# dohlee/chromoformer

Measured on AMD Instinct MI355X. Metric: genes/sec training (bsz=64, default config), higher is better.
Workload: dtype f32

## Files before the change

chromoformer_amd/csrc/cf_attc1.h:

```cpp
#pragma once

namespace cf {

__host__ __device__ inline size_t attc1_smem(int L, int F) {
    const int Lpad = attc2_lpad(L);
    return (size_t)(2 * kD + 16 + 16 + kD * 8 + ((L * F + 8 + 3) & ~3) + 2 * (Lpad + 4) + 2 * Lpad + 64 + 16 * 2 * kD) * sizeof(float) + (size_t)Lpad;
}

#define CF_STAMP1(slot)                                                                                   \
    do {                                                                                                  \
        if (a.tdbg && stamp_wg == 0 && threadIdx.x == 0)                                                   \
            a.tdbg[(BWD ? 16 : 0) + (slot)] = __builtin_amdgcn_s_memtime();                               \
    } while (0)
template <bool BWD>
__device__ __forceinline__ void attc1_body(const Attc2Args& a, const int r, const int n, float* smem, const int stamp_wg = -1) {
    const int tid = threadIdx.x;
    const int w = tid >> 6, lane = tid & 63;
    const int L = a.L[r], Lpad = a.Lpad[r], LT = a.LT[r], F = a.F, LS = Lpad + 4;
    float* vin_s = smem;
    float* u_s = vin_s + 2 * kD;
    float* w_s = u_s + 16;
    float* wlp_s = w_s + 16;
    float* feats_s = wlp_s + kD * 8;
    float* sc_s = feats_s + ((L * F + 8 + 3) & ~3);
    float* p_s = sc_s + 2 * LS;
    float* red_s = p_s + 2 * Lpad;
    float* part_s = red_s + 64;
    uint8_t* mk_s = reinterpret_cast<uint8_t*>(part_s + 16 * 2 * kD);

    CF_STAMP1(0);
    const int eg = tid >> 7, j4 = tid & 127;
    float4 tb[16];
    {
        const float* fg = a.feats[r] + (size_t)n * L * F;
        const uint8_t* mg = a.mask[r] + (size_t)n * a.mstride[r];
        const float wl0 = (tid & 7) < F ? ldg(a.wlp[r] + (tid >> 3) * F + (tid & 7)) : 0.f;
        const float wl1 = (tid & 7) < F ? ldg(a.wlp[r] + ((tid + kAT) >> 3) * F + (tid & 7)) : 0.f;
        float4 vv = make_float4(0.f, 0.f, 0.f, 0.f);
        if (tid < 64) vv = ldg4(a.vin[r] + (size_t)n * 256 + tid * 4);
        uint8_t mb[2];
#pragma unroll
        for (int u = 0; u < 2; ++u) {
            const int j = tid + u * kAT;
            mb[u] = *(const CF_GLOBAL uint8_t*)(mg + min(j, L - 1));
        }
        float pb[4];
        if (BWD) {
            const float* pg = a.p[r] + (size_t)n * 2 * L;
#pragma unroll
            for (int u = 0; u < 4; ++u) {
                const int i = tid + u * kAT, h = i / Lpad, j = i - h * Lpad;
                pb[u] = ldg(pg + min(h, 1) * L + min(j, L - 1));
            }
        }
        float fb[8];
        const int nfe = L * F;
#pragma unroll
        for (int u = 0; u < 8; ++u) fb[u] = ldg(fg + min(tid + u * kAT, nfe - 1));
        {
            const float* pt = a.pet[r] + (size_t)(eg * 32) * LT + min(4 * j4, LT - 4);
#pragma unroll
            for (int k = 0; k < 16; ++k) tb[k] = ldg4(pt + (size_t)k * LT);
        }
        __builtin_amdgcn_sched_barrier(0);
        wlp_s[tid] = wl0;
        wlp_s[tid + kAT] = wl1;
        if (tid < 64) *reinterpret_cast<float4*>(vin_s + tid * 4) = vv;
#pragma unroll
        for (int u = 0; u < 2; ++u)
            if (tid + u * kAT < Lpad) mk_s[tid + u * kAT] = tid + u * kAT < L ? mb[u] : (uint8_t)1;
        if (BWD)
#pragma unroll
            for (int u = 0; u < 4; ++u)
                if (tid + u * kAT < 2 * Lpad) p_s[tid + u * kAT] = (tid + u * kAT) % Lpad < L ? pb[u] : 0.f;
#pragma unroll
        for (int u = 0; u < 8; ++u)
            if (tid + u * kAT < nfe + 8) feats_s[tid + u * kAT] = tid + u * kAT < nfe ? fb[u] : 0.f;
        for (int i = tid + 8 * kAT; i < nfe + 8; i += kAT) feats_s[i] = i < nfe ? ldg(fg + i) : 0.f;
        for (int i = tid; i < 2 * LS; i += kAT) {
            const int j = i % LS;
            if (j >= L) sc_s[i] = 0.f;
        }
    }
    __syncthreads();
    CF_STAMP1(1);
    {
        const int o = tid >> 5, part = tid & 31, h = o >> 3, f = o & 7;
        float acc = 0.f;
#pragma unroll
        for (int i = 0; i < 4; ++i) acc = fmaf(vin_s[h * kD + part * 4 + i], wlp_s[(part * 4 + i) * 8 + f], acc);
        acc = group16_sum(acc);
        acc += __shfl_xor(acc, 16, 64);
        if (part == 0) u_s[o] = acc;
    }
    float t0[2] = {0.f, 0.f}, t1[2] = {0.f, 0.f};
    for (int c = 0; c * kAT < L; ++c) {
        const int jc = min(c * kAT + 4 * j4, LT - 4);
        const float* pt = a.pet[r] + (size_t)(eg * 32) * LT + jc;
        float4 s0 = make_float4(0.f, 0.f, 0.f, 0.f), s1 = s0;
#pragma unroll
        for (int half = 0; half < 2; ++half) {
            float4 b[16];
            if (c == 0) {
#pragma unroll
                for (int k = 0; k < 16; ++k) b[k] = tb[k];
                if (half == 0) {
#pragma unroll
                    for (int k = 0; k < 16; ++k) tb[k] = ldg4(pt + (size_t)(16 + k) * LT);
                }
            } else {
#pragma unroll
                for (int k = 0; k < 16; ++k) b[k] = ldg4(pt + (size_t)(half * 16 + k) * LT);
            }
#pragma unroll
            for (int k4 = 0; k4 < 4; ++k4) {
                const float4 v0 = *reinterpret_cast<const float4*>(vin_s + eg * 32 + half * 16 + 4 * k4);
                const float4 v1 = *reinterpret_cast<const float4*>(vin_s + kD + eg * 32 + half * 16 + 4 * k4);
                const float q0[4] = {v0.x, v0.y, v0.z, v0.w}, q1[4] = {v1.x, v1.y, v1.z, v1.w};
#pragma unroll
                for (int i = 0; i < 4; ++i) {
                    const float4 bb = b[4 * k4 + i];
                    s0 = make_float4(fmaf(q0[i], bb.x, s0.x), fmaf(q0[i], bb.y, s0.y), fmaf(q0[i], bb.z, s0.z), fmaf(q0[i], bb.w, s0.w));
                    s1 = make_float4(fmaf(q1[i], bb.x, s1.x), fmaf(q1[i], bb.y, s1.y), fmaf(q1[i], bb.z, s1.z), fmaf(q1[i], bb.w, s1.w));
                }
            }
        }
        if (c) __syncthreads();
        *reinterpret_cast<float4*>(part_s + (eg * 2) * kAT + 4 * j4) = s0;
        *reinterpret_cast<float4*>(part_s + (eg * 2 + 1) * kAT + 4 * j4) = s1;
        __syncthreads();
        t0[c] = (part_s[tid] + part_s[2 * kAT + tid]) + (part_s[4 * kAT + tid] + part_s[6 * kAT + tid]);
        t1[c] = (part_s[kAT + tid] + part_s[3 * kAT + tid]) + (part_s[5 * kAT + tid] + part_s[7 * kAT + tid]);
    }
    const int e4 = tid & 31, jg = tid >> 5;
    const int per5 = (L + 15) / 16;
    const int j05 = jg * per5, nj5 = max(0, min(L, j05 + per5) - j05);
    const float* pp5 = a.pe[r] + (size_t)min(j05, Lpad - 1) * kD + 4 * e4;
#pragma unroll
    for (int k = 0; k < 16; ++k) tb[k] = ldg4(pp5 + (size_t)min(k, max(nj5 - 1, 0)) * kD);
    __syncthreads();
    CF_STAMP1(2);
    auto block_reduce = [&](float v0, float v1, bool is_max, float& o0, float& o1) {
        v0 = is_max ? wave_max(v0) : wave_sum(v0);
        v1 = is_max ? wave_max(v1) : wave_sum(v1);
        __syncthreads();
        if (lane == 0) {
            red_s[w * 2] = v0;
            red_s[w * 2 + 1] = v1;
        }
        __syncthreads();
        o0 = red_s[0];
        o1 = red_s[1];
#pragma unroll
        for (int k = 1; k < kAT / 64; ++k) {
            o0 = is_max ? fmaxf(o0, red_s[k * 2]) : o0 + red_s[k * 2];
            o1 = is_max ? fmaxf(o1, red_s[k * 2 + 1]) : o1 + red_s[k * 2 + 1];
        }
    };
    {
        float x0[2], x1[2];
        bool valid[2], masked[2];
#pragma unroll
        for (int c = 0; c < 2; ++c) {
            const int j = tid + c * kAT;
            valid[c] = j < L;
            masked[c] = valid[c] && mk_s[min(j, Lpad - 1)];
            float f0 = 0.f, f1 = 0.f;
// ... 31 lines not shown
            const float r0 = 1.0f / Z0, r1 = 1.0f / Z1;
            float* pg = a.p[r] + (size_t)n * 2 * L;
#pragma unroll
            for (int c = 0; c < 2; ++c) {
                const int j = tid + c * kAT;
                if (valid[c]) {
                    const float p0 = x0[c] * r0, p1 = x1[c] * r1;
                    sc_s[j] = p0;
                    sc_s[LS + j] = p1;
                    stg(pg + j, p0);
                    stg(pg + L + j, p1);
                }
            }
        } else {
            float d0 = 0.f, d1 = 0.f;
#pragma unroll
            for (int c = 0; c < 2; ++c) {
                const int j = tid + c * kAT;
                if (valid[c]) {
                    d0 = fmaf(p_s[j], x0[c], d0);
                    d1 = fmaf(p_s[Lpad + j], x1[c], d1);
                }
            }
            float D0, D1;
            block_reduce(d0, d1, false, D0, D1);
#pragma unroll
            for (int c = 0; c < 2; ++c) {
                const int j = tid + c * kAT;
                if (valid[c]) {
                    sc_s[j] = masked[c] ? 0.f : p_s[j] * (x0[c] - D0) * a.rscale;
                    sc_s[LS + j] = masked[c] ? 0.f : p_s[Lpad + j] * (x1[c] - D1) * a.rscale;
                }
            }
        }
    }
    __syncthreads();
    CF_STAMP1(3);
    {
        const int o = tid >> 5, part = tid & 31, h = o >> 3, f = o & 7;
        float acc = 0.f;
        if (f < F)
            for (int j = part; j < L; j += 32) acc = fmaf(sc_s[h * LS + j], feats_s[(size_t)j * F + f], acc);
        acc = group16_sum(acc);
        acc += __shfl_xor(acc, 16, 64);
        if (part == 0) {
            w_s[o] = acc;
            stg(a.w[r] + (size_t)n * 16 + o, acc);
        }
    }
    CF_STAMP1(4);
    CF_STAMP1(5);
    {
        float4 o0 = make_float4(0.f, 0.f, 0.f, 0.f), o1 = o0;
        for (int jb = 0; jb < nj5; jb += 16) {
            float4 b[16];
#pragma unroll
            for (int k = 0; k < 16; ++k) b[k] = tb[k];
            if (jb + 16 < nj5) {
#pragma unroll
                for (int k = 0; k < 16; ++k) tb[k] = ldg4(pp5 + (size_t)min(jb + 16 + k, nj5 - 1) * kD);
            }
#pragma unroll
            for (int k = 0; k < 16; ++k) {
                const bool in = jb + k < nj5;
                const float ph = in ? sc_s[j05 + jb + k] : 0.f, qh = in ? sc_s[LS + j05 + jb + k] : 0.f;
                o0 = make_float4(fmaf(ph, b[k].x, o0.x), fmaf(ph, b[k].y, o0.y), fmaf(ph, b[k].z, o0.z), fmaf(ph, b[k].w, o0.w));
                o1 = make_float4(fmaf(qh, b[k].x, o1.x), fmaf(qh, b[k].y, o1.y), fmaf(qh, b[k].z, o1.z), fmaf(qh, b[k].w, o1.w));
            }
        }
        __syncthreads();
        *reinterpret_cast<float4*>(part_s + (jg * 2) * kD + 4 * e4) = o0;
        *reinterpret_cast<float4*>(part_s + (jg * 2 + 1) * kD + 4 * e4) = o1;
    }
    __syncthreads();
    CF_STAMP1(6);
    if (tid < 2 * kD) {
        const int h = tid >> 7, e = tid & 127;
        float v = 0.f;
#pragma unroll
        for (int g = 0; g < 16; ++g) v += part_s[(g * 2 + h) * kD + e];
#pragma unroll
        for (int f = 0; f < 8; ++f) v = fmaf(w_s[h * 8 + f], wlp_s[e * 8 + f], v);
        stg(a.vout[r] + (size_t)n * 256 + tid, v);
    }
    CF_STAMP1(7);
}
template <bool BWD>
__global__ __launch_bounds__(kAT) void k_attc1(Attc2Args a) {
    extern __shared__ __attribute__((aligned(16))) float smem[];
    attc1_body<BWD>(a, gridDim.y - 1 - blockIdx.y, blockIdx.x, smem, blockIdx.y * gridDim.x + blockIdx.x);
}

}
```

chromoformer_amd/csrc/cf_attc2.h:

```cpp
#pragma once
#include <type_traits>

namespace cf {

struct Attc2Args {
    const float* feats[kMaxRes];
    const uint8_t* mask[kMaxRes];
    long long mstride[kMaxRes];
    const float* pe[kMaxRes];
    const float* pet[kMaxRes];
    const float* wlp[kMaxRes];
    const float* vin[kMaxRes];
    float* p[kMaxRes];
    float* w[kMaxRes];
    float* vout[kMaxRes];
    int L[kMaxRes], Lpad[kMaxRes], LT[kMaxRes];
    int N, F;
    float scale, rscale;
    unsigned long long* tdbg;
    unsigned long long* tall;
};
#define CF_STAMP2(slot)                                                                                   \
    do {                                                                                                  \
        if (a.tdbg && stamp_wg == 0 && (threadIdx.x & 63) == 0)                                            \
// ... 9 lines not shown

__device__ __forceinline__ void frag_load_nn_rt(FragNN<4, 8>& f, const float* __restrict__ Bm, int ldb, int nchunks) {
    const int lane = threadIdx.x & 63, r = lane & 15, q = lane >> 4;
    f.bp = Bm + (size_t)(q * 4) * ldb + 4 * r;
    f.ldb = ldb;
#pragma unroll
    for (int c = 0; c < kRing - 1; ++c) frag_chunk_nn(f, c, min(c, nchunks - 1));
    __builtin_amdgcn_sched_barrier(0);
}
__device__ __forceinline__ void frag_mma_nn_rt(FragNN<4, 8>& f, const float* As, int lda, int nchunks, f32x4 (&acc)[4]) {
    const int lane = threadIdx.x & 63, r = lane & 15, q = lane >> 4;
    const float* ap = As + r * lda + q * 4;
    float4 a_nxt = *reinterpret_cast<const float4*>(ap);
    for (int c0 = 0; c0 < nchunks; c0 += kRing) {
#pragma unroll
        for (int u = 0; u < kRing; ++u) {
            const int c = c0 + u;
            if (c + kRing - 1 < nchunks) frag_chunk_nn(f, (u + kRing - 1) % kRing, c + kRing - 1);
            __builtin_amdgcn_sched_barrier(0);
            if (c < nchunks)
#pragma unroll
                for (int k = 0; k < 2; ++k) {
                    const float4 a = a_nxt;
                    a_nxt = *reinterpret_cast<const float4*>(ap + (c * 2 + k + 1) * 16);
                    const float av[4] = {a.x, a.y, a.z, a.w};
#pragma unroll
                    for (int i = 0; i < 4; ++i) {
                        const float* bv = reinterpret_cast<const float*>(&f.ring[u][k][i]);
#pragma unroll
                        for (int t = 0; t < 4; ++t) acc[t] = mfma4(av[i], bv[t], acc[t]);
                    }
                }
        }
    }
}

__host__ __device__ inline size_t attc2_scratch_floats(int L) { return (size_t)kTile * (attc2_lpad(L) + 4) + 2 * kTile * (kD + 4) + 2 * kTile * 8; }
__host__ __device__ inline size_t attc2_persist_bytes(int L, int F, int AG) {
    return (size_t)(kD * 8 + AG * L * F + 8) * sizeof(float) + (size_t)AG * attc2_lpad(L);
}
template <int AG>
__device__ __forceinline__ void attc2_stage(const float* feats, const uint8_t* mask, long long mstride, const float* wlp, int L, int Lpad, int F,
                                            const int n0, const int N, float* persist) {
    const int tid = threadIdx.x, w = __builtin_amdgcn_readfirstlane(tid >> 6);
    float* wlp_s = persist;
    float* feats_s = wlp_s + kD * 8;
    uint8_t* mk_s = reinterpret_cast<uint8_t*>(feats_s + AG * L * F + 8);
    const int nreg = min(AG, N - n0);
    const float* fg = feats + (size_t)n0 * L * F;
    const int nf = nreg * L * F;
    constexpr int NFL = AG == 8 ? 12 : AG == 4 ? 6 : AG == 2 ? 3 : 2;
    const bool f16b = ((L * F) & 3) == 0 && AG * L * F <= NFL * 4 * kAT && (reinterpret_cast<uintptr_t>(fg) & 15) == 0;
    if (f16b) {
        const int n4 = (AG * L * F) >> 2, last4 = (nf >> 2) - 1;
#pragma unroll
        for (int u = 0; u < NFL; ++u) {
            const int i = tid + u * kAT;
            typedef __attribute__((address_space(3))) void* lds_void;
            typedef const __attribute__((address_space(1))) void* glb_void;
            if (i < n4)
                __builtin_amdgcn_global_load_lds((glb_void)(fg + (size_t)min(i, last4) * 4), (lds_void)(feats_s + (size_t)(w * 64 + u * kAT) * 4), 16, 0, 0);
        }
    } else {
        for (int i = tid; i < AG * L * F; i += kAT) feats_s[i] = i < nf ? ldg(fg + i) : 0.f;
    }
    if (tid < 8) feats_s[AG * L * F + tid] = 0.f;
    static_assert(kD * 8 == 2 * kAT, "wlp staging assumes two entries per thread");
    wlp_s[tid] = (tid & 7) < F ? ldg(wlp + (tid >> 3) * F + (tid & 7)) : 0.f;
    wlp_s[tid + kAT] = (tid & 7) < F ? ldg(wlp + ((tid + kAT) >> 3) * F + (tid & 7)) : 0.f;
    const uint8_t* mg = mask + (size_t)n0 * mstride;
    const bool words = ((L | (int)mstride | (int)(reinterpret_cast<uintptr_t>(mask))) & 3) == 0;
    if (words) {
        const int LW = Lpad >> 2, lw = L >> 2;
        uint32_t* mk_w = reinterpret_cast<uint32_t*>(mk_s);
        for (int idx = tid; idx < AG * LW; idx += kAT) {
            const int sreg = idx / LW, jw = idx - sreg * LW;
            mk_w[idx] = (sreg < nreg && jw < lw) ? *(const CF_GLOBAL uint32_t*)(mg + (size_t)sreg * mstride + 4 * jw) : 0x01010101u;
        }
    } else {
        for (int s = 0; s < AG; ++s)
            for (int j = tid; j < Lpad; j += kAT) mk_s[s * Lpad + j] = (s < nreg && j < L) ? *(const CF_GLOBAL uint8_t*)(mg + (size_t)s * mstride + j) : (uint8_t)1;
    }
}
template <bool BWD, int AG, bool STAGED = false>
__device__ __forceinline__ void attc2_body(const Attc2Args& a, const int r, const int n0, const int N, float* scratch, float* persist,
                                           const int stamp_wg = -1) {
    constexpr int kAG = AG;
    const int tid = threadIdx.x;
    const int w = tid >> 6, lane = tid & 63, lr = lane & 15, lq = lane >> 4;
    const int L = a.L[r], Lpad = a.Lpad[r], LT = a.LT[r], F = a.F, LS = Lpad + 4;
    constexpr int LD = kD + 4, NW = kAT / 64;
    float* sc_s = scratch;
    float* vin_s = sc_s + kTile * LS;
    float* red_s = vin_s + kTile * LD;
    float* u_s = red_s + kTile * LD;
    float* w_s = u_s + kTile * 8;
    float* wlp_s = persist;
    float* feats_s = wlp_s + kD * 8;
    uint8_t* mk_s = reinterpret_cast<uint8_t*>(feats_s + kAG * L * F + 8);
    const int nreg = min(kAG, N - n0);

    CF_STAMP2(0);
    if (a.tall && tid == 0 && stamp_wg >= 0) a.tall[stamp_wg * 2] = __builtin_amdgcn_s_memtime();
    const int nblk = (L + 63) / 64;
    float* stat_s = red_s;
    static_assert(2 * kTile * 16 <= kTile * LD, "statistics fit in the K-split partial buffer");
    FragNN<4, 8> ft0;
    const float* fg = a.feats[r] + (size_t)n0 * L * F;
    const int nf = nreg * L * F;
    constexpr int NFL = AG == 8 ? 12 : AG == 4 ? 6 : AG == 2 ? 3 : 2;
    const bool f16b = ((L * F) & 3) == 0 && kAG * L * F <= NFL * 4 * kAT;
    float4 fv12[NFL];
    {
        const uint8_t* mg = a.mask[r] + (size_t)n0 * a.mstride[r];
        const bool words = ((L | (int)a.mstride[r] | (int)(reinterpret_cast<uintptr_t>(a.mask[r]))) & 3) == 0;
        const int LW = Lpad >> 2, lw = L >> 2;
        constexpr int MW = kAG >= 2 ? kAG / 2 : 1;
        float4 vv = make_float4(0.f, 0.f, 0.f, 0.f);
        {
            const int m = tid >> 5, c4 = tid & 31;
            if ((m >> 1) < nreg) vv = ldg4(a.vin[r] + (size_t)n0 * 256 + m * kD + c4 * 4);
        }
        const float wl0 = !STAGED && (tid & 7) < F ? ldg(a.wlp[r] + (tid >> 3) * F + (tid & 7)) : 0.f;
        const float wl1 = !STAGED && (tid & 7) < F ? ldg(a.wlp[r] + ((tid + kAT) >> 3) * F + (tid & 7)) : 0.f;
        uint32_t mwv[MW];
        if (!STAGED && words) {
#pragma unroll
            for (int k = 0; k < MW; ++k) {
                const int idx = tid + k * kAT, sreg = idx / LW, jw = idx - sreg * LW;
                mwv[k] = (idx < kAG * LW && sreg < nreg && jw < lw) ? *(const CF_GLOBAL uint32_t*)(mg + (size_t)sreg * a.mstride[r] + 4 * jw) : 0x01010101u;
            }
        }
        {
            if (!STAGED) {
                const float* fa = reinterpret_cast<const float*>(reinterpret_cast<uintptr_t>(fg) & ~(uintptr_t)15);
                const int last4 = f16b ? (nf >> 2) - 1 : max((nf >> 2) - 2, 0);
#pragma unroll
                for (int u = 0; u < NFL; ++u) fv12[u] = ldg4(fa + (size_t)min(tid + u * kAT, last4) * 4);
            }
            const float* bm_ = a.pet[r] + min(w, nblk - 1) * 64;
            ft0.bp = bm_ + (size_t)(lq * 4) * LT + 4 * lr;
            ft0.ldb = LT;
            frag_chunk_nn(ft0, 0, 0);
        }
        __builtin_amdgcn_sched_barrier(0);
        stat_s[tid] = tid < kTile * 16 ? 0.f : -INFINITY;
        if (tid < kTile) u_s[tid * 8 + 7] = 0.f;
        {
            const int m = tid >> 5;
            for (int j = L + (tid & 31); j < Lpad; j += 32) sc_s[m * LS + j] = 0.f;
        }
        *reinterpret_cast<float4*>(vin_s + (tid >> 5) * LD + (tid & 31) * 4) = vv;
        static_assert(kD * 8 == 2 * kAT, "wlp staging assumes two entries per thread");
        if (!STAGED) {
            wlp_s[tid] = wl0;
            wlp_s[tid + kAT] = wl1;
        }
        if (STAGED) {
        } else if (words) {
            uint32_t* mk_w = reinterpret_cast<uint32_t*>(mk_s);
#pragma unroll
            for (int k = 0; k < MW; ++k)
                if (tid + k * kAT < kAG * LW) mk_w[tid + k * kAT] = mwv[k];
        } else {
            for (int s = 0; s < kAG; ++s)
                for (int j = tid; j < Lpad; j += kAT)
// ... 375 lines not shown
```

chromoformer_amd/csrc/cf_trunk.h:

```cpp
#pragma once

namespace cf {

constexpr int kMaxPairLayers = 4;

struct CentreLayerDev {
    const float *wq_t, *wk, *wv_t, *wo_t, *bo, *g1, *be1, *w1_t, *b1, *w2_t, *b2, *g2, *be2;
    const float *wq, *wk_t, *wv, *wo, *w1, *w2;
    float *q, *qt, *p, *w, *xbar, *a, *xh1, *rs1, *y1, *hdn, *xh2, *rs2, *out, *xin;
    float *dt2, *dpre1, *dt1, *da, *dxbar, *dqt, *du, *dq, *dx, *partial;
};
struct TrunkResDev {
    CentreLayerDev E, P[kMaxPairLayers];
    const float *pe, *pe2, *pet2;
    const float *wlp_e, *wlp_p;
    const float *lin_p_t, *lin_p;
    float *ex0, *featc, *xp0, *dxp0, *edout, *rx0, *drx0;
    float *lp_part_e, *lp_part_p;
    int L, Lpad, LT, pad_;
};
struct TrunkArgs {
    const TrunkResDev* tab;
    const float* pfeats[kMaxRes];
    const uint8_t* pmask[kMaxRes];
    long long pmstride[kMaxRes];
    const float* cfeats[kMaxRes];
    const uint8_t* cmask[kMaxRes];
    long long cmstride[kMaxRes];
    const float* dhin;
    int B, S, T, F, n_res, pair_layers, save;
    float scale, rscale;
    const RetileUnit* rt_units;
    const float* rt_params;
    float* rt_tiled;
    float* rt_tiledT;
    int rt_n;
    RecordArgs rec;
    int* adv_cursor;
    const LpJob* lp_jobs;
    const WgTile* rd_tiles;
    int rd_n, rd_batch;
    AdamFuse rd_opt;
    unsigned long long* tdbg;
};

template <class T>
__device__ __forceinline__ T ldc(const T* p) {
    static_assert(sizeof(T) == 8 || sizeof(T) == 4, "pointer or int fields");
    if constexpr (sizeof(T) == 8) {
        const unsigned long long v = *(const __attribute__((address_space(4))) unsigned long long*)p;
        return __builtin_bit_cast(T, v);
    } else {
        const unsigned v = *(const __attribute__((address_space(4))) unsigned*)p;
        return __builtin_bit_cast(T, v);
    }
}
#define TF(field) ldc(&R->field)

__host__ __device__ inline size_t trunk_scratch_floats(int L, int dff_max) {
    const size_t chain = (size_t)3 * kTile * (kD + 4) + (size_t)kTile * ((dff_max > 256 ? dff_max : 256) + 4);
    const size_t att = attc2_scratch_floats(L);
    return (chain > att ? chain : att) + 4;
}
__host__ __device__ inline size_t trunk_smem(int L, int F, int dff_max) {
    const size_t two = trunk_scratch_floats(L, dff_max) * sizeof(float) + attc2_persist_bytes(L, F, kAGMax);
    const size_t one = attc1_smem(L, F);
    const size_t rt = (size_t)(kAT / 64) * 16 * 20 * sizeof(float);
    const size_t lp = (size_t)80 * (kD + 8) * sizeof(float);
    size_t m = two > one ? two : one;
    m = m > rt ? m : rt;
    return m > lp ? m : lp;
}

#ifndef CF_STAMP_Y
#define CF_STAMP_Y 0
#endif
#define CF_PHASE static __device__ __forceinline__

struct TrunkCtx {
    const TrunkResDev* R;
    const float* feats;
    const uint8_t* mask;
    long long mstride;
    int g, S, T, F, save;
    float scale, rscale;
};
__device__ __forceinline__ void launder(TrunkCtx& c, float*& smem, float*& persist) {
    asm volatile("" : "+s"(c.R), "+s"(c.feats), "+s"(c.mask), "+s"(c.mstride), "+s"(c.g), "+s"(c.S), "+s"(c.T), "+s"(c.F), "+s"(c.save),
                 "+s"(c.scale), "+s"(c.rscale));
    typedef __attribute__((address_space(3))) float* lds_ptr;
    unsigned a = (unsigned)(uintptr_t)(lds_ptr)smem, b = (unsigned)(uintptr_t)(lds_ptr)persist;
    asm volatile("" : "+s"(a), "+s"(b));
    smem = (float*)(lds_ptr)(uintptr_t)a;
    persist = (float*)(lds_ptr)(uintptr_t)b;
}
__device__ __forceinline__ void trunk_attc_args(Attc2Args& at, const TrunkCtx& c, const float* wlp, const float* vin, float* p, float* w, float* vout,
                                                int N) {
    const TrunkResDev* R = c.R;
    at.feats[0] = c.feats;
    at.mask[0] = c.mask;
    at.mstride[0] = c.mstride;
    at.pe[0] = TF(pe2);
    at.pet[0] = TF(pet2);
    at.wlp[0] = wlp;
    at.vin[0] = vin;
    at.p[0] = p;
    at.w[0] = w;
    at.vout[0] = vout;
    at.L[0] = TF(L);
    at.Lpad[0] = TF(Lpad);
    at.LT[0] = TF(LT);
    at.N = N;
    at.F = c.F;
    at.scale = c.scale;
    at.rscale = c.rscale;
    at.tdbg = nullptr;
    at.tall = nullptr;
}
#define CF_CHAIN_TILES(scratch)                                                                       \
    float (*xs)[kD + 4] = reinterpret_cast<float (*)[kD + 4]>(scratch);                               \
    float (*as_)[kD + 4] = reinterpret_cast<float (*)[kD + 4]>((scratch) + kTile * (kD + 4));         \
    float (*ts)[kD + 4] = reinterpret_cast<float (*)[kD + 4]>((scratch) + 2 * kTile * (kD + 4));      \
    float* wide_raw = (scratch) + 3 * kTile * (kD + 4);                                               \
    (void)xs, (void)as_, (void)ts, (void)wide_raw

}
#include "cf_trunk_e.h"
namespace cf {

template <bool BWD>
CF_PHASE void trunk_attc1_e(TrunkCtx c, float* smem) {
    const TrunkResDev* R = c.R;
    Attc2Args at;
    if (!BWD) trunk_attc_args(at, c, TF(wlp_e), TF(E.qt), TF(E.p), TF(E.w), TF(E.xbar), c.g + 1);
    else trunk_attc_args(at, c, TF(wlp_e), TF(E.dxbar), TF(E.p), TF(E.du), TF(E.dqt), c.g + 1);
    attc1_body<BWD>(at, 0, c.g, smem);
}
__device__ __forceinline__ void trunk_post_args(PostArgs& po, const CentreLayerDev* P, int save) {
    po.ain[0] = ldc(&P->xbar);
    po.wv[0] = ldc(&P->wv_t);
    po.wo[0] = ldc(&P->wo_t);
    po.bo[0] = ldc(&P->bo);
    po.g1[0] = ldc(&P->g1);
    po.be1[0] = ldc(&P->be1);
    po.w1[0] = ldc(&P->w1_t);
    po.b1[0] = ldc(&P->b1);
    po.w2[0] = ldc(&P->w2_t);
    po.b2[0] = ldc(&P->b2);
    po.g2[0] = ldc(&P->g2);
    po.be2[0] = ldc(&P->be2);
    po.a_out[0] = ldc(&P->a);
    po.xh1[0] = ldc(&P->xh1);
    po.rs1[0] = ldc(&P->rs1);
    po.y1[0] = ldc(&P->y1);
    po.hdn[0] = ldc(&P->hdn);
    po.xh2[0] = ldc(&P->xh2);
    po.rs2[0] = ldc(&P->rs2);
    po.save = save;
    po.lin_w[0] = nullptr;
    po.nq_wq[0] = nullptr;
}
CF_PHASE void trunk_qchain_p0(TrunkCtx c, float* smem) {
    const TrunkResDev* R = c.R;
    CF_CHAIN_TILES(smem);
    const CentreLayerDev* P0 = &R->P[0];
    QChainArgs q;
    q.x[0] = TF(xp0);
    q.xmap = RowMap{c.S, 1, 0, 0};
    q.wq[0] = ldc(&P0->wq_t);
    q.wk[0] = ldc(&P0->wk);
    q.q[0] = ldc(&P0->q);
    q.qt[0] = ldc(&P0->qt);
    q.xcopy[0] = ldc(&P0->xin);
    q.N = c.g * c.S + c.S;
    qchain_fwd_body<kAT / 64>(q, 0, c.g * c.S, xs, as_);
}
template <bool BWD, bool STAGED>
CF_PHASE void trunk_attc2_p(TrunkCtx c, int l, float* scratch, float* persist) {
    const TrunkResDev* R = c.R;
    const CentreLayerDev* P = &R->P[l];
    const int row0 = c.g * c.S, NB = row0 + c.S;
    Attc2Args at;
    if (!BWD) trunk_attc_args(at, c, TF(wlp_p), ldc(&P->qt), ldc(&P->p), ldc(&P->w), ldc(&P->xbar), NB);
    else trunk_attc_args(at, c, TF(wlp_p), ldc(&P->dxbar), ldc(&P->p), ldc(&P->du), ldc(&P->dqt), NB);
    attc2_body<BWD, kAGMax, STAGED>(at, 0, row0, NB, scratch, persist);
}
CF_PHASE void trunk_stage_p(TrunkCtx c, float* persist) {
    const TrunkResDev* R = c.R;
    attc2_stage<kAGMax>(c.feats, c.mask, c.mstride, TF(wlp_p), TF(L), TF(Lpad), c.F, c.g * c.S, c.g * c.S + c.S, persist);
}
template <int DFF>
CF_PHASE void trunk_post_p(TrunkCtx c, int l, int n_layers, float* smem) {
    const TrunkResDev* R = c.R;
    const CentreLayerDev* P = &R->P[l];
    const bool last = l + 1 == n_layers;
    const int S = c.S, row0 = c.g * S, NB = row0 + S;
    CF_CHAIN_TILES(smem);
    PostArgs po;
    trunk_post_args(po, P, c.save);
    po.x[0] = l == 0 ? (const float*)TF(xp0) : (const float*)ldc(&R->P[l > 0 ? l - 1 : 0].out);
    po.xmap = l == 0 ? RowMap{S, 1, 0, 0} : identity_map();
    po.out[0] = last ? TF(rx0) : ldc(&P->out);
    po.omap = last ? RowMap{S, c.T, 1, 1} : identity_map();
    po.N = NB;
    if (!last) {
        const CentreLayerDev* Pn = &R->P[l + 1];
        po.nq_wq[0] = ldc(&Pn->wq_t);
        po.nq_wk[0] = ldc(&Pn->wk);
        po.nq_q[0] = ldc(&Pn->q);
        po.nq_qt[0] = ldc(&Pn->qt);
    }
    post_fwd_body<true, 128, DFF, kAT / 64>(po, 0, row0, NB, xs, as_, ts, reinterpret_cast<float (*)[PostFwdLds<DFF>::HW + 4]>(wide_raw));
}

template <int DFF_E, int DFF_P, int PL>
__global__ __launch_bounds__(kAT) void k_trunk_fwd(TrunkArgs a) {
    extern __shared__ __attribute__((aligned(16))) float smem[];
    constexpr int NWV = kAT / 64;
    if ((int)blockIdx.y >= a.n_res) {
        float (*tp)[16][20] = reinterpret_cast<float (*)[16][20]>(smem);
        for (int u = blockIdx.x; u < a.rt_n; u += gridDim.x) {
            retile_unit_lds<NWV>(a.rt_params, a.rt_tiled, a.rt_tiledT, a.rt_units[u], tp);
            __syncthreads();
        }
        return;
    }
    if (a.adv_cursor && blockIdx.x == 0 && blockIdx.y == 0 && threadIdx.x == 0 && a.adv_cursor[0] < a.adv_cursor[1]) a.adv_cursor[0] += 1;
    const int r = a.n_res - 1 - (int)blockIdx.y;
    const TrunkResDev* R = a.tab + r;
    constexpr int DFF_MAX = DFF_E > DFF_P ? DFF_E : DFF_P;
    float* sm = smem;
    float* persist = smem + trunk_scratch_floats(TF(L), DFF_MAX);
    TrunkCtx c{R, a.pfeats[r], a.pmask[r], a.pmstride[r], (int)blockIdx.x, a.S, a.T, a.F, a.save, a.scale, a.rscale};
    int stamp_i = 0;
    if (a.tdbg && blockIdx.x == 0 && blockIdx.y == CF_STAMP_Y && threadIdx.x == 0) a.tdbg[stamp_i++] = __builtin_amdgcn_s_memtime();
#define CF_NEXT_PHASE                                                                                     \
    __syncthreads();                                                                                      \
    if (a.tdbg && blockIdx.x == 0 && blockIdx.y == CF_STAMP_Y && threadIdx.x == 0) a.tdbg[stamp_i++] = __builtin_amdgcn_s_memtime(); \
    launder(c, sm, persist)
    {
        TrunkCtx cs{R, a.cfeats[r], a.cmask[r], a.cmstride[r], (int)blockIdx.x, a.S, a.T, a.F, a.save, a.scale, a.rscale};
        trunk_stage_p(cs, persist);
        launder(c, sm, persist);
    }
    trunk_e_front(c, sm);
    CF_NEXT_PHASE;
    trunk_attc1_e<false>(c, sm);
    CF_NEXT_PHASE;
    trunk_e_post_fwd<DFF_E>(c, sm);
    c.feats = a.cfeats[r];
    c.mask = a.cmask[r];
    c.mstride = a.cmstride[r];
    CF_NEXT_PHASE;
    trunk_qchain_p0(c, sm);
    asm volatile("s_waitcnt vmcnt(0)" ::: "memory");
    CF_NEXT_PHASE;
    trunk_attc2_p<false, true>(c, 0, sm, persist);
    CF_NEXT_PHASE;
    trunk_post_p<DFF_P>(c, 0, PL, sm);
#pragma unroll
    for (int l = 1; l < PL; ++l) {
        CF_NEXT_PHASE;
        trunk_attc2_p<false, true>(c, l, sm, persist);
        CF_NEXT_PHASE;
        trunk_post_p<DFF_P>(c, l, PL, sm);
    }
    CF_NEXT_PHASE;
}

__device__ __forceinline__ void trunk_post_bwd_args(PostBwdArgs& pb, const CentreLayerDev* P) {
    pb.xh2[0] = ldc(&P->xh2);
    pb.rs2[0] = ldc(&P->rs2);
    pb.g2[0] = ldc(&P->g2);
    pb.hdn[0] = ldc(&P->hdn);
    pb.w2[0] = ldc(&P->w2);
    pb.w1[0] = ldc(&P->w1);
    pb.xh1[0] = ldc(&P->xh1);
    pb.rs1[0] = ldc(&P->rs1);
    pb.g1[0] = ldc(&P->g1);
    pb.wo[0] = ldc(&P->wo);
    pb.wv[0] = ldc(&P->wv);
    pb.dt2[0] = ldc(&P->dt2);
    pb.dpre1[0] = ldc(&P->dpre1);
    pb.dt1[0] = ldc(&P->dt1);
    pb.da[0] = ldc(&P->da);
    pb.dxbar[0] = ldc(&P->dxbar);
    pb.partial[0] = ldc(&P->partial);
}
#define CF_BWD_TILES(DFF)                                                                                       \
    constexpr int WW_ = (DFF) > 128 ? (DFF) : 128;                                                              \
    float (*wide)[WW_ + 4] = reinterpret_cast<float (*)[WW_ + 4]>(wide_raw)
template <int DFF>
CF_PHASE void trunk_post_bwd_p(TrunkCtx c, int l, int n_layers, float* smem) {
    const TrunkResDev* R = c.R;
    const CentreLayerDev* P = &R->P[l];
    const bool last = l + 1 == n_layers;
    const int S = c.S, row0 = c.g * S, NB = row0 + S;
    CF_CHAIN_TILES(smem);
    CF_BWD_TILES(DFF);
    PostBwdArgs pb;
    trunk_post_bwd_args(pb, P);
    pb.dout[0] = last ? (const float*)TF(drx0) : (const float*)ldc(&R->P[last ? l : l + 1].dx);
    pb.dmap = last ? RowMap{S, c.T, 1, 1} : identity_map();
    pb.N = NB;
    post_bwd_body<true, 128, DFF, kAT / 64>(pb, 0, row0, NB, c.g, xs, as_, ts, wide);
}
CF_PHASE void trunk_qchain_bwd(TrunkCtx c, const CentreLayerDev* P, int row0, int NB, float* smem) {
    float (*ds)[256 + 4] = reinterpret_cast<float (*)[256 + 4]>(smem);
    float (*qs)[kD + 4] = reinterpret_cast<float (*)[kD + 4]>(smem + kTile * (256 + 4));
    QBwdArgs qb;
    qb.dqt[0] = ldc(&P->dqt);
    qb.dres[0] = ldc(&P->dt1);
    qb.wk[0] = ldc(&P->wk_t);
    qb.wq[0] = ldc(&P->wq);
    qb.dq[0] = ldc(&P->dq);
    qb.dx[0] = ldc(&P->dx);
    qb.N = NB;
    (void)c;
    qchain_bwd_body<kAT / 64>(qb, 0, row0, ds, qs);
}
CF_PHASE void trunk_join(TrunkCtx c, const float* dhin, int r, int n_res, float* smem) {
    const TrunkResDev* R = c.R;
    const int g = c.g, S = c.S, tid = threadIdx.x;
    float* xk = smem;
    float* red = smem + kD;
    if (tid < kD) {
        const float* dxp = ldc(&R->P[0].dx) + (size_t)g * S * kD + tid;
        float s = 0.f;
        for (int i = 0; i < S; ++i) s += ldg(dxp + (size_t)i * kD);
        xk[tid] = s;
        stg(TF(dxp0) + (size_t)g * kD + tid, s);
    }
// ... 138 lines not shown
```

chromoformer_amd/csrc/cf_trunk_e.h:

```cpp
#pragma once

namespace cf {

static_assert(kAT == kMvT, "the one-row products of cf_valu_mv.h are laid out for the trunk's workgroup size");

constexpr int kEvX = 0;
constexpr int kEvB = 128;
constexpr int kEvA = 384;
constexpr int kEvT = 512;
constexpr int kEvH = 640;
constexpr int kEvX2 = 896;
constexpr int kEvW = 1024;
constexpr int kEvW2 = 2048;
constexpr int kEvP = 3072;
constexpr int kEvEnd = kEvP + 16 * 256;

CF_PHASE void trunk_e_front(TrunkCtx c, float* smem) {
    const TrunkResDev* R = c.R;
    const int g = c.g, tid = threadIdx.x;
    float* xs = smem + kEvX;
    float* qs = smem + kEvA;
    float* part = smem + kEvP;
    NtW<kD, kD> wq;
    nt_request(wq, TF(E.wq_t));
    TrW<kD, kD> wk;
    tr_request(wk, TF(E.wk));
    __builtin_amdgcn_sched_barrier(0);
    if (tid < kD) {
        const int L = TF(L), cb = L / 2, F = c.F;
        const float* f = c.feats + ((size_t)g * L + cb) * F;
        const float* wl = TF(wlp_e) + tid * F;
        float acc = 0.f;
        for (int i = 0; i < F; ++i) acc = fmaf(ldg(f + i), ldg(wl + i), acc);
        const float x = acc + ldg(TF(pe) + (size_t)cb * kD + tid);
        xs[tid] = x;
        stg(TF(ex0) + (size_t)g * kD + tid, x);
        if (tid < 8) stg(TF(featc) + (size_t)g * 8 + tid, tid < F ? ldg(f + tid) : 0.f);
    }
    __syncthreads();
    {
        float q[1];
        nt_dot(wq, xs, q);
        if (nt_writer()) {
            const int n = nt_row<kD, kD>(0);
            qs[n] = q[0];
            stg(TF(E.q) + (size_t)g * kD + n, q[0]);
        }
    }
    __syncthreads();
    tr_partial(wk, qs, part);
    __syncthreads();
    if (tid < 2 * kD) {
        const int h = tid >> 7, e = tid & (kD - 1);
        stg(TF(E.qt) + (size_t)g * 2 * kD + tid, tr_sum<kD>(part, h * 8, 8, e));
    }
}

template <int DFF>
CF_PHASE void trunk_e_post_fwd(TrunkCtx c, float* smem) {
    const TrunkResDev* R = c.R;
    const int g = c.g, tid = threadIdx.x, w = tid >> 6, lane = tid & 63;
    const bool save = c.save != 0;
    float* xs = smem + kEvX;
    float* xb = smem + kEvB;
    float* as_ = smem + kEvA;
    float* ts = smem + kEvT;
    float* hs = smem + kEvH;
    float* y1w = smem + kEvW + w * kD;
    float* ow = smem + kEvW2 + w * kD;
    static_assert(DFF == 128 || DFF == 256, "hidden width of the Embedding layer");
    NtW<kD, kD> wv, wo;
    nt_request(wv, TF(E.wv_t));
    float rx = 0.f, rb = 0.f;
    if (tid < kD) rx = ldg(TF(ex0) + (size_t)g * kD + tid);
    if (tid < 2 * kD) rb = ldg(TF(E.xbar) + (size_t)g * 2 * kD + tid);
    nt_request(wo, TF(E.wo_t));
    const int n = nt_row<kD, kD>(0);
    const float g1a = ldg(TF(E.g1) + lane), g1b = ldg(TF(E.g1) + lane + 64), b1a = ldg(TF(E.be1) + lane), b1b = ldg(TF(E.be1) + lane + 64);
    const float g2a = ldg(TF(E.g2) + lane), g2b = ldg(TF(E.g2) + lane + 64), b2a = ldg(TF(E.be2) + lane), b2b = ldg(TF(E.be2) + lane + 64);
    const float bo = ldg(TF(E.bo) + n), b2 = ldg(TF(E.b2) + n);
    __builtin_amdgcn_sched_barrier(0);
    if (tid < kD) xs[tid] = rx;
    if (tid < 2 * kD) xb[tid] = rb;
    __syncthreads();
    {
        float a[1];
        nt_dot(wv, xb + (n >> 6) * kD, a);
        if (nt_writer()) {
            as_[n] = a[0];
            if (save) stg(TF(E.a) + (size_t)g * kD + n, a[0]);
        }
    }
    NtW<DFF, kD> w1;
    nt_request(w1, TF(E.w1_t));
    __builtin_amdgcn_sched_barrier(0);
    __syncthreads();
    {
        float t[1];
        nt_dot(wo, as_, t);
        if (nt_writer()) ts[n] = t[0] + bo + xs[n];
    }
    NtW<kD, DFF> w2;
    nt_request(w2, TF(E.w2_t));
    float b1[NtW<DFF, kD>::TW];
#pragma unroll
    for (int t = 0; t < NtW<DFF, kD>::TW; ++t) b1[t] = ldg(TF(E.b1) + nt_row<DFF, kD>(t));
    __builtin_amdgcn_sched_barrier(0);
    __syncthreads();
    {
        const LnRow o = ln_row_fwd(ts[lane], ts[lane + 64], g1a, g1b, b1a, b1b);
        y1w[lane] = o.y0;
        y1w[lane + 64] = o.y1;
        if (w == 0 && save) {
            stg(TF(E.xh1) + (size_t)g * kD + lane, o.x0);
            stg(TF(E.xh1) + (size_t)g * kD + lane + 64, o.x1);
            stg(TF(E.y1) + (size_t)g * kD + lane, o.y0);
            stg(TF(E.y1) + (size_t)g * kD + lane + 64, o.y1);
            if (lane == 0) stg(TF(E.rs1) + g, o.rstd);
        }
    }
    __builtin_amdgcn_wave_barrier();
    {
        float v[NtW<DFF, kD>::TW];
        nt_dot(w1, y1w, v);
        if (nt_writer())
#pragma unroll
            for (int t = 0; t < NtW<DFF, kD>::TW; ++t) {
                const int j = nt_row<DFF, kD>(t);
                const float hv = fmaxf(v[t] + b1[t], 0.f);
                hs[j] = hv;
                if (save) stg(TF(E.hdn) + (size_t)g * DFF + j, hv);
            }
    }
    NtW<kD, kD> wl;
    nt_request(wl, TF(lin_p_t));
    __builtin_amdgcn_sched_barrier(0);
    __syncthreads();
    {
        float t[1];
        nt_dot(w2, hs, t);
        if (nt_writer()) ts[n] = t[0] + b2 + y1w[n];
    }
    __syncthreads();
    {
        const LnRow o = ln_row_fwd(ts[lane], ts[lane + 64], g2a, g2b, b2a, b2b);
        ow[lane] = o.y0;
        ow[lane + 64] = o.y1;
        if (w == 0) {
            if (save) {
                stg(TF(E.xh2) + (size_t)g * kD + lane, o.x0);
                stg(TF(E.xh2) + (size_t)g * kD + lane + 64, o.x1);
                if (lane == 0) stg(TF(E.rs2) + g, o.rstd);
            }
            float* rx0 = TF(rx0) + (size_t)g * c.T * kD;
            stg(rx0 + lane, o.y0);
            stg(rx0 + lane + 64, o.y1);
        }
    }
    __builtin_amdgcn_wave_barrier();
    {
        float v[1];
        nt_dot(wl, ow, v);
        if (nt_writer()) stg(TF(xp0) + (size_t)g * kD + n, v[0]);
    }
}

template <int DFF>
// ... 124 lines not shown
```

Measured before the change: 130,600.

## Stage attention inputs during embedding front and hand over state in LDS

The embedding-front phase now issues the global loads for the following attc1 and attc2 phases (features, masks, projection weights, with async global-to-LDS copies where alignment allows) and writes them into a persistent LDS handover region. The attc1 forward pass reads its staged features and mask from there, skips its own load and barrier, and writes its output vector into LDS. The post phase reads x0 and xbar from LDS instead of reloading them from global memory. This hides load latency behind front-phase compute and removes global round trips between phases, at the cost of more shared memory per workgroup and higher register pressure in the front phase.

```diff
diff --git a/chromoformer_amd/csrc/cf_attc1.h b/chromoformer_amd/csrc/cf_attc1.h
--- a/chromoformer_amd/csrc/cf_attc1.h
+++ b/chromoformer_amd/csrc/cf_attc1.h
@@ -12,8 +12,38 @@
         if (a.tdbg && stamp_wg == 0 && threadIdx.x == 0)                                                   \
             a.tdbg[(BWD ? 16 : 0) + (slot)] = __builtin_amdgcn_s_memtime();                               \
     } while (0)
-template <bool BWD>
-__device__ __forceinline__ void attc1_body(const Attc2Args& a, const int r, const int n, float* smem, const int stamp_wg = -1) {
+struct Attc1Staged {
+    float wl0, wl1, fb[8];
+    uint8_t mb[2];
+};
+__device__ __forceinline__ void attc1_stage_req(Attc1Staged& st, const float* fg, const uint8_t* mg, const float* wlp, const int L, const int F) {
+    const int tid = threadIdx.x, nfe = L * F;
+    st.wl0 = (tid & 7) < F ? ldg(wlp + (tid >> 3) * F + (tid & 7)) : 0.f;
+    st.wl1 = (tid & 7) < F ? ldg(wlp + ((tid + kAT) >> 3) * F + (tid & 7)) : 0.f;
+#pragma unroll
+    for (int u = 0; u < 2; ++u) st.mb[u] = *(const CF_GLOBAL uint8_t*)(mg + min(tid + u * kAT, L - 1));
+#pragma unroll
+    for (int u = 0; u < 8; ++u) st.fb[u] = ldg(fg + min(tid + u * kAT, nfe - 1));
+}
+__device__ __forceinline__ void attc1_stage_put(const Attc1Staged& st, const float* fg, const int L, const int Lpad, const int F, float* wlp_s,
+                                                float* feats_s, uint8_t* mk_s) {
+    const int tid = threadIdx.x, nfe = L * F;
+    wlp_s[tid] = st.wl0;
+    wlp_s[tid + kAT] = st.wl1;
+#pragma unroll
+    for (int u = 0; u < 2; ++u)
+        if (tid + u * kAT < Lpad) mk_s[tid + u * kAT] = tid + u * kAT < L ? st.mb[u] : (uint8_t)1;
+#pragma unroll
+    for (int u = 0; u < 8; ++u)
+        if (tid + u * kAT < nfe + 8) feats_s[tid + u * kAT] = tid + u * kAT < nfe ? st.fb[u] : 0.f;
+    for (int i = tid + 8 * kAT; i < nfe + 8; i += kAT) feats_s[i] = i < nfe ? ldg(fg + i) : 0.f;
+}
+__host__ __device__ inline size_t attc1_staged_floats(int L, int F) { return (size_t)((L * F + 8 + 3) & ~3) + (size_t)attc2_lpad(L) / 4; }
+
+template <bool BWD, bool STAGED = false>
+__device__ __forceinline__ void attc1_body(const Attc2Args& a, const int r, const int n, float* smem, const int stamp_wg = -1, float* staged = nullptr,
+                                           float* vout_s = nullptr) {
+    static_assert(!(BWD && STAGED), "only the forward is staged");
     const int tid = threadIdx.x;
     const int w = tid >> 6, lane = tid & 63;
     const int L = a.L[r], Lpad = a.Lpad[r], LT = a.LT[r], F = a.F, LS = Lpad + 4;
@@ -21,17 +51,27 @@
     float* u_s = vin_s + 2 * kD;
     float* w_s = u_s + 16;
     float* wlp_s = w_s + 16;
-    float* feats_s = wlp_s + kD * 8;
-    float* sc_s = feats_s + ((L * F + 8 + 3) & ~3);
+    float* feats_own = wlp_s + kD * 8;
+    float* feats_s = STAGED ? staged : feats_own;
+    float* sc_s = feats_own + ((L * F + 8 + 3) & ~3);
     float* p_s = sc_s + 2 * LS;
     float* red_s = p_s + 2 * Lpad;
     float* part_s = red_s + 64;
-    uint8_t* mk_s = reinterpret_cast<uint8_t*>(part_s + 16 * 2 * kD);
+    uint8_t* mk_s = reinterpret_cast<uint8_t*>(STAGED ? staged + ((L * F + 8 + 3) & ~3) : part_s + 16 * 2 * kD);
 
     CF_STAMP1(0);
     const int eg = tid >> 7, j4 = tid & 127;
     float4 tb[16];
-    {
+    if constexpr (STAGED) {
+        const float* pt = a.pet[r] + (size_t)(eg * 32) * LT + min(4 * j4, LT - 4);
+#pragma unroll
+        for (int k = 0; k < 16; ++k) tb[k] = ldg4(pt + (size_t)k * LT);
+        __builtin_amdgcn_sched_barrier(0);
+        for (int i = tid; i < 2 * LS; i += kAT) {
+            const int j = i % LS;
+            if (j >= L) sc_s[i] = 0.f;
+        }
+    } else {
         const float* fg = a.feats[r] + (size_t)n * L * F;
         const uint8_t* mg = a.mask[r] + (size_t)n * a.mstride[r];
         const float wl0 = (tid & 7) < F ? ldg(a.wlp[r] + (tid >> 3) * F + (tid & 7)) : 0.f;
@@ -82,7 +122,7 @@
             if (j >= L) sc_s[i] = 0.f;
         }
     }
-    __syncthreads();
+    if (!STAGED) __syncthreads();
     CF_STAMP1(1);
     {
         const int o = tid >> 5, part = tid & 31, h = o >> 3, f = o & 7;
@@ -280,6 +320,7 @@
 #pragma unroll
         for (int f = 0; f < 8; ++f) v = fmaf(w_s[h * 8 + f], wlp_s[e * 8 + f], v);
         stg(a.vout[r] + (size_t)n * 256 + tid, v);
+        if (STAGED) vout_s[tid] = v;
     }
     CF_STAMP1(7);
 }
diff --git a/chromoformer_amd/csrc/cf_attc2.h b/chromoformer_amd/csrc/cf_attc2.h
--- a/chromoformer_amd/csrc/cf_attc2.h
+++ b/chromoformer_amd/csrc/cf_attc2.h
@@ -115,6 +115,79 @@
             for (int j = tid; j < Lpad; j += kAT) mk_s[s * Lpad + j] = (s < nreg && j < L) ? *(const CF_GLOBAL uint8_t*)(mg + (size_t)s * mstride + j) : (uint8_t)1;
     }
 }
+template <int AG>
+struct Attc2Staged {
+    static constexpr int MW = AG >= 2 ? AG / 2 : 1;
+    float wl0, wl1;
+    uint32_t mw[MW];
+};
+template <int AG>
+__device__ __forceinline__ void attc2_stage_req(Attc2Staged<AG>& st, const float* feats, const uint8_t* mask, long long mstride, const float* wlp, int L,
+                                                int Lpad, int F, const int n0, const int N, float* persist) {
+    const int tid = threadIdx.x, w = __builtin_amdgcn_readfirstlane(tid >> 6);
+    float* feats_s = persist + kD * 8;
+    const int nreg = min(AG, N - n0);
+    const float* fg = feats + (size_t)n0 * L * F;
+    const int nf = nreg * L * F;
+    constexpr int NFL = AG == 8 ? 12 : AG == 4 ? 6 : AG == 2 ? 3 : 2;
+    const bool f16b = ((L * F) & 3) == 0 && AG * L * F <= NFL * 4 * kAT && (reinterpret_cast<uintptr_t>(fg) & 15) == 0;
+    st.wl0 = (tid & 7) < F ? ldg(wlp + (tid >> 3) * F + (tid & 7)) : 0.f;
+    st.wl1 = (tid & 7) < F ? ldg(wlp + ((tid + kAT) >> 3) * F + (tid & 7)) : 0.f;
+    const uint8_t* mg = mask + (size_t)n0 * mstride;
+    const bool words = ((L | (int)mstride | (int)(reinterpret_cast<uintptr_t>(mask))) & 3) == 0;
+    const int LW = Lpad >> 2, lw = L >> 2;
+#pragma unroll
+    for (int k = 0; k < Attc2Staged<AG>::MW; ++k) {
+        const int idx = min(tid + k * kAT, AG * LW - 1), sreg = min(idx / LW, nreg - 1), jw = min(idx - (idx / LW) * LW, max(lw - 1, 0));
+        st.mw[k] = words ? *(const CF_GLOBAL uint32_t*)(mg + (size_t)sreg * mstride + 4 * jw) : 0u;
+    }
+    __builtin_amdgcn_sched_barrier(0);
+    if (f16b) {
+        const int n4 = (AG * L * F) >> 2, last4 = (nf >> 2) - 1;
+#pragma unroll
+        for (int u = 0; u < NFL; ++u) {
+            const int i = tid + u * kAT;
+            typedef __attribute__((address_space(3))) void* lds_void;
+            typedef const __attribute__((address_space(1))) void* glb_void;
+            if (i < n4)
+                __builtin_amdgcn_global_load_lds((glb_void)(fg + (size_t)min(i, last4) * 4), (lds_void)(feats_s + (size_t)(w * 64 + u * kAT) * 4), 16, 0, 0);
+        }
+    }
+    __builtin_amdgcn_sched_barrier(0);
+}
+template <int AG>
+__device__ __forceinline__ void attc2_stage_put(const Attc2Staged<AG>& st, const float* feats, const uint8_t* mask, long long mstride, int L, int Lpad,
+                                                int F, const int n0, const int N, float* persist) {
+    const int tid = threadIdx.x;
+    float* wlp_s = persist;
+    float* feats_s = wlp_s + kD * 8;
+    uint8_t* mk_s = reinterpret_cast<uint8_t*>(feats_s + AG * L * F + 8);
+    const int nreg = min(AG, N - n0);
+    const float* fg = feats + (size_t)n0 * L * F;
+    const int nf = nreg * L * F;
+    constexpr int NFL = AG == 8 ? 12 : AG == 4 ? 6 : AG == 2 ? 3 : 2;
+    const bool f16b = ((L * F) & 3) == 0 && AG * L * F <= NFL * 4 * kAT && (reinterpret_cast<uintptr_t>(fg) & 15) == 0;
+    static_assert(kD * 8 == 2 * kAT, "wlp staging assumes two entries per thread");
+    wlp_s[tid] = st.wl0;
+    wlp_s[tid + kAT] = st.wl1;
+    if (tid < 8) feats_s[AG * L * F + tid] = 0.f;
+    const uint8_t* mg = mask + (size_t)n0 * mstride;
+    const bool words = ((L | (int)mstride | (int)(reinterpret_cast<uintptr_t>(mask))) & 3) == 0;
+    if (words) {
+        const int LW = Lpad >> 2, lw = L >> 2;
+        uint32_t* mk_w = reinterpret_cast<uint32_t*>(mk_s);
+#pragma unroll
+        for (int k = 0; k < Attc2Staged<AG>::MW; ++k) {
+            const int idx = tid + k * kAT, sreg = idx / LW, jw = idx - sreg * LW;
+            if (idx < AG * LW) mk_w[idx] = (sreg < nreg && jw < lw) ? st.mw[k] : 0x01010101u;
+        }
+    } else {
+        for (int s = 0; s < AG; ++s)
+            for (int j = tid; j < Lpad; j += kAT) mk_s[s * Lpad + j] = (s < nreg && j < L) ? *(const CF_GLOBAL uint8_t*)(mg + (size_t)s * mstride + j) : (uint8_t)1;
+    }
+    if (!f16b)
+        for (int i = tid; i < AG * L * F; i += kAT) feats_s[i] = i < nf ? ldg(fg + i) : 0.f;
+}
 template <bool BWD, int AG, bool STAGED = false>
 __device__ __forceinline__ void attc2_body(const Attc2Args& a, const int r, const int n0, const int N, float* scratch, float* persist,
                                            const int stamp_wg = -1) {
diff --git a/chromoformer_amd/csrc/cf_trunk.h b/chromoformer_amd/csrc/cf_trunk.h
--- a/chromoformer_amd/csrc/cf_trunk.h
+++ b/chromoformer_amd/csrc/cf_trunk.h
@@ -57,13 +57,17 @@
 }
 #define TF(field) ldc(&R->field)
 
+constexpr int kHoXb = 0;
+constexpr int kHoX0 = 2 * kD;
+constexpr int kHoStrip = 3 * kD;
+__host__ __device__ inline size_t trunk_handover_floats(int L, int F) { return (size_t)kHoStrip + attc1_staged_floats(L, F); }
 __host__ __device__ inline size_t trunk_scratch_floats(int L, int dff_max) {
     const size_t chain = (size_t)3 * kTile * (kD + 4) + (size_t)kTile * ((dff_max > 256 ? dff_max : 256) + 4);
     const size_t att = attc2_scratch_floats(L);
     return (chain > att ? chain : att) + 4;
 }
 __host__ __device__ inline size_t trunk_smem(int L, int F, int dff_max) {
-    const size_t two = trunk_scratch_floats(L, dff_max) * sizeof(float) + attc2_persist_bytes(L, F, kAGMax);
+    const size_t two = trunk_scratch_floats(L, dff_max) * sizeof(float) + attc2_persist_bytes(L, F, kAGMax) + trunk_handover_floats(L, F) * sizeof(float);
     const size_t one = attc1_smem(L, F);
     const size_t rt = (size_t)(kAT / 64) * 16 * 20 * sizeof(float);
     const size_t lp = (size_t)80 * (kD + 8) * sizeof(float);
@@ -129,12 +133,13 @@
 namespace cf {
 
 template <bool BWD>
-CF_PHASE void trunk_attc1_e(TrunkCtx c, float* smem) {
+CF_PHASE void trunk_attc1_e(TrunkCtx c, float* smem, float* ho = nullptr) {
     const TrunkResDev* R = c.R;
     Attc2Args at;
     if (!BWD) trunk_attc_args(at, c, TF(wlp_e), TF(E.qt), TF(E.p), TF(E.w), TF(E.xbar), c.g + 1);
     else trunk_attc_args(at, c, TF(wlp_e), TF(E.dxbar), TF(E.p), TF(E.du), TF(E.dqt), c.g + 1);
-    attc1_body<BWD>(at, 0, c.g, smem);
+    if constexpr (BWD) attc1_body<true>(at, 0, c.g, smem);
+    else attc1_body<false, true>(at, 0, c.g, smem, -1, ho + kHoStrip, ho + kHoXb);
 }
 __device__ __forceinline__ void trunk_post_args(PostArgs& po, const CentreLayerDev* P, int save) {
     po.ain[0] = ldc(&P->xbar);
@@ -238,16 +243,15 @@
     __syncthreads();                                                                                      \
     if (a.tdbg && blockIdx.x == 0 && blockIdx.y == CF_STAMP_Y && threadIdx.x == 0) a.tdbg[stamp_i++] = __builtin_amdgcn_s_memtime(); \
     launder(c, sm, persist)
+#define CF_HANDOVER (persist + attc2_persist_bytes(ldc(&c.R->L), c.F, kAGMax) / sizeof(float))
     {
         TrunkCtx cs{R, a.cfeats[r], a.cmask[r], a.cmstride[r], (int)blockIdx.x, a.S, a.T, a.F, a.save, a.scale, a.rscale};
-        trunk_stage_p(cs, persist);
-        launder(c, sm, persist);
-    }
-    trunk_e_front(c, sm);
-    CF_NEXT_PHASE;
-    trunk_attc1_e<false>(c, sm);
-    CF_NEXT_PHASE;
-    trunk_e_post_fwd<DFF_E>(c, sm);
+        trunk_e_front(c, cs, sm, persist, CF_HANDOVER);
+    }
+    CF_NEXT_PHASE;
+    trunk_attc1_e<false>(c, sm, CF_HANDOVER);
+    CF_NEXT_PHASE;
+    trunk_e_post_fwd<DFF_E>(c, sm, CF_HANDOVER);
     c.feats = a.cfeats[r];
     c.mask = a.cmask[r];
     c.mstride = a.cmstride[r];
diff --git a/chromoformer_amd/csrc/cf_trunk_e.h b/chromoformer_amd/csrc/cf_trunk_e.h
--- a/chromoformer_amd/csrc/cf_trunk_e.h
+++ b/chromoformer_amd/csrc/cf_trunk_e.h
@@ -15,28 +15,51 @@
 constexpr int kEvP = 3072;
 constexpr int kEvEnd = kEvP + 16 * 256;
 
-CF_PHASE void trunk_e_front(TrunkCtx c, float* smem) {
+constexpr int kEvFront = 2 * kD + 32 + kD * 8;
+CF_PHASE void trunk_e_front(TrunkCtx c, TrunkCtx cs, float* smem, float* persist, float* ho) {
     const TrunkResDev* R = c.R;
     const int g = c.g, tid = threadIdx.x;
-    float* xs = smem + kEvX;
-    float* qs = smem + kEvA;
-    float* part = smem + kEvP;
+    float* xs = smem + kEvFront + kEvX;
+    float* qs = smem + kEvFront + kEvA;
+    float* part = smem + kEvFront + kEvP;
+    const int L = TF(L), Lpad = TF(Lpad), cb = L / 2, F = c.F;
     NtW<kD, kD> wq;
     nt_request(wq, TF(E.wq_t));
     TrW<kD, kD> wk;
     tr_request(wk, TF(E.wk));
-    __builtin_amdgcn_sched_barrier(0);
+    const float* f = c.feats + ((size_t)g * L + cb) * F;
+    const float* wl = TF(wlp_e) + (tid & (kD - 1)) * F;
+    float fv[8], wv[8];
+#pragma unroll
+    for (int i = 0; i < 8; ++i) {
+        fv[i] = ldg(f + min(i, F - 1));
+        wv[i] = ldg(wl + min(i, F - 1));
+    }
+    const float pec = ldg(TF(pe) + (size_t)cb * kD + (tid & (kD - 1)));
+    const float* fge = c.feats + (size_t)g * L * F;
+    Attc1Staged se;
+    attc1_stage_req(se, fge, c.mask + (size_t)g * c.mstride, TF(wlp_e), L, F);
+    Attc2Staged<kAGMax> sp;
+    attc2_stage_req<kAGMax>(sp, cs.feats, cs.mask, cs.mstride, TF(wlp_p), L, Lpad, F, g * c.S, g * c.S + c.S, persist);
     if (tid < kD) {
-        const int L = TF(L), cb = L / 2, F = c.F;
-        const float* f = c.feats + ((size_t)g * L + cb) * F;
-        const float* wl = TF(wlp_e) + tid * F;
         float acc = 0.f;
-        for (int i = 0; i < F; ++i) acc = fmaf(ldg(f + i), ldg(wl + i), acc);
-        const float x = acc + ldg(TF(pe) + (size_t)cb * kD + tid);
+#pragma unroll
+        for (int i = 0; i < 8; ++i)
+            if (i < F) acc = fmaf(fv[i], wv[i], acc);
+        const float x = acc + pec;
         xs[tid] = x;
+        ho[kHoX0 + tid] = x;
         stg(TF(ex0) + (size_t)g * kD + tid, x);
-        if (tid < 8) stg(TF(featc) + (size_t)g * 8 + tid, tid < F ? ldg(f + tid) : 0.f);
-    }
+        if (tid < 8) {
+            float fc = 0.f;
+#pragma unroll
+            for (int i = 0; i < 8; ++i)
+                if (i == tid && i < F) fc = fv[i];
+            stg(TF(featc) + (size_t)g * 8 + tid, fc);
+        }
+    }
+    attc1_stage_put(se, fge, L, Lpad, F, smem + 2 * kD + 32, ho + kHoStrip, reinterpret_cast<uint8_t*>(ho + kHoStrip + ((L * F + 8 + 3) & ~3)));
+    attc2_stage_put<kAGMax>(sp, cs.feats, cs.mask, cs.mstride, L, Lpad, F, g * c.S, g * c.S + c.S, persist);
     __syncthreads();
     {
         float q[1];
@@ -52,17 +75,19 @@
     __syncthreads();
     if (tid < 2 * kD) {
         const int h = tid >> 7, e = tid & (kD - 1);
-        stg(TF(E.qt) + (size_t)g * 2 * kD + tid, tr_sum<kD>(part, h * 8, 8, e));
+        const float v = tr_sum<kD>(part, h * 8, 8, e);
+        stg(TF(E.qt) + (size_t)g * 2 * kD + tid, v);
+        smem[tid] = v;
     }
 }
 
 template <int DFF>
-CF_PHASE void trunk_e_post_fwd(TrunkCtx c, float* smem) {
+CF_PHASE void trunk_e_post_fwd(TrunkCtx c, float* smem, const float* ho) {
     const TrunkResDev* R = c.R;
     const int g = c.g, tid = threadIdx.x, w = tid >> 6, lane = tid & 63;
     const bool save = c.save != 0;
-    float* xs = smem + kEvX;
-    float* xb = smem + kEvB;
+    const float* xs = ho + kHoX0;
+    const float* xb = ho + kHoXb;
     float* as_ = smem + kEvA;
     float* ts = smem + kEvT;
     float* hs = smem + kEvH;
@@ -71,18 +96,12 @@
     static_assert(DFF == 128 || DFF == 256, "hidden width of the Embedding layer");
     NtW<kD, kD> wv, wo;
     nt_request(wv, TF(E.wv_t));
-    float rx = 0.f, rb = 0.f;
-    if (tid < kD) rx = ldg(TF(ex0) + (size_t)g * kD + tid);
-    if (tid < 2 * kD) rb = ldg(TF(E.xbar) + (size_t)g * 2 * kD + tid);
     nt_request(wo, TF(E.wo_t));
     const int n = nt_row<kD, kD>(0);
     const float g1a = ldg(TF(E.g1) + lane), g1b = ldg(TF(E.g1) + lane + 64), b1a = ldg(TF(E.be1) + lane), b1b = ldg(TF(E.be1) + lane + 64);
     const float g2a = ldg(TF(E.g2) + lane), g2b = ldg(TF(E.g2) + lane + 64), b2a = ldg(TF(E.be2) + lane), b2b = ldg(TF(E.be2) + lane + 64);
     const float bo = ldg(TF(E.bo) + n), b2 = ldg(TF(E.b2) + n);
     __builtin_amdgcn_sched_barrier(0);
-    if (tid < kD) xs[tid] = rx;
-    if (tid < 2 * kD) xb[tid] = rb;
-    __syncthreads();
     {
         float a[1];
         nt_dot(wv, xb + (n >> 6) * kD, a);
```

New measurement: 131,300, median of 6. About the same (+0.5%).
